# ethz-asl/laser_slam

Hardware: NVIDIA B200
Metric: ICP registrations/s (131072-pt scan vs 524288-pt map, 30 iterations) (higher is better)
Workload: dtype f32

## Files before the change

laser_slam_b200/csrc/ls_api.cu:

```cuda
#include <cstdarg>
#include <cstddef>
#include <cstdio>
#include <cstdlib>
#include <cstring>
#include <string>
#include <utility>
#include <vector>

#include "../../include/ls_b200.h"
#include "ls_kernels.cuh"

using namespace ls;

#define LS_VERSION 100

struct Workspace {
  cudaStream_t stream = nullptr;
  cudaEvent_t ev0 = nullptr, ev1 = nullptr, ev2 = nullptr, ev_launch = nullptr;
  int n_cap = 0, m_cap = 0, cells_cap = 0, tab_cap = 0, hist_cap = 0;
  BuildArrays A{};
  BuildState* bs = nullptr;
  float4 *reading = nullptr, *rd = nullptr;
  float4 *ref_stage = nullptr, *ref_nrm_stage = nullptr;
  float* nrm_raw = nullptr;
// ... 126 lines not shown
    if ((rc = dev_alloc(ctx, &w->ids, (size_t)cap))) return rc;
    if ((rc = dev_alloc(ctx, &w->d2_out, (size_t)cap))) return rc;
    if ((rc = dev_alloc(ctx, &w->A.qkey, (size_t)cap))) return rc;
    if ((rc = dev_alloc(ctx, &w->A.qperm, (size_t)cap))) return rc;
    if ((rc = dev_alloc(ctx, &w->A.rd_s, (size_t)cap))) return rc;
    w->n_cap = cap;
  }
  if (m > w->m_cap) {
    const int cap = m + m / 8 + 1024;
    int rc;
    if ((rc = dev_alloc(ctx, &w->A.sub_pts, (size_t)cap))) return rc;
    if ((rc = dev_alloc(ctx, &w->A.sub_nrm, (size_t)cap))) return rc;
    if ((rc = dev_alloc(ctx, &w->A.srt_pts, (size_t)cap))) return rc;
    if ((rc = dev_alloc(ctx, &w->A.srt_nrm, (size_t)cap))) return rc;
    if ((rc = dev_alloc(ctx, &w->A.pkey, (size_t)cap))) return rc;
    if ((rc = dev_alloc(ctx, &w->ref_stage, (size_t)cap))) return rc;
    if ((rc = dev_alloc(ctx, &w->ref_nrm_stage, (size_t)cap))) return rc;
    int tcap = cap / 17 + 1024;
    const int tmax = (int)((size_t)1536 * 1024 * 1024 / ((size_t)LS_FB3 * 12));
    if (tcap > tmax) tcap = tmax;
    if ((rc = dev_alloc(ctx, &w->A.tab1, (size_t)tcap * LS_FB3))) return rc;
    if ((rc = dev_alloc(ctx, &w->A.cnt1, (size_t)tcap * LS_FB3))) return rc;
    if ((rc = dev_alloc(ctx, &w->A.tab1_cell, (size_t)tcap))) return rc;
    if ((rc = dev_alloc(ctx, &w->A.qtab_local, (size_t)tcap * LS_FB3))) return rc;
    if ((rc = dev_alloc(ctx, &w->A.qtab_total, (size_t)tcap))) return rc;
    CU(cudaMemsetAsync(w->A.cnt1, 0, (size_t)tcap * LS_FB3 * sizeof(uint32_t), w->stream));
    w->stream_dirty = true;
    w->A.tab_cap = tcap;
    w->tab_cap = tcap;
    w->m_cap = cap;
  }
  if (max_cells > w->cells_cap) {
    int rc;
    if ((rc = dev_alloc(ctx, &w->A.top, (size_t)max_cells + 1))) return rc;
    if ((rc = dev_alloc(ctx, &w->A.cnt0, (size_t)max_cells + 1))) return rc;
    if ((rc = dev_alloc(ctx, &w->A.pyr, (size_t)max_cells / 2 + 4096))) return rc;
    if ((rc = dev_alloc(ctx, &w->A.topmask, (size_t)max_cells + 1))) return rc;
    if ((rc = dev_alloc(ctx, &w->A.qtop_start, (size_t)max_cells + 1))) return rc;
    CU(cudaMemsetAsync(w->A.cnt0, 0, ((size_t)max_cells + 1) * sizeof(uint32_t), w->stream));
    w->stream_dirty = true;
    w->cells_cap = max_cells;
  }
  if (max_iter > w->hist_cap) {
    int rc;
    if ((rc = dev_alloc(ctx, &w->T_hist, (size_t)max_iter * 16))) return rc;
    w->hist_cap = max_iter;
  }
  return LS_OK;
}

struct Resolved {
  float cell;
  int split, max_cells;
};

Resolved resolve(const ls_icp_params* p) {
  Resolved r;
  r.cell = p->cell_size > 0.f ? p->cell_size : 1.0f;
  r.split = p->leaf_split > 0 ? (p->leaf_split < 16 ? 16 : p->leaf_split) : 32;
  r.max_cells = p->max_cells > 0 ? p->max_cells : (1 << 22);
  if (r.max_cells > (1 << 22)) r.max_cells = 1 << 22;
  if (r.max_cells < 64) r.max_cells = 64;
  return r;
}

int check_params(ls_ctx* ctx, const ls_icp_params* p) {
  if (!p) return fail(ctx, LS_ERR_ARG, "null params");
  if (p->max_iterations < 1 || p->max_iterations > 100000) return fail(ctx, LS_ERR_ARG, "max_iterations out of range");
  if (!(p->trim_ratio > 0.f) || p->trim_ratio > 1.f) return fail(ctx, LS_ERR_ARG, "trim_ratio must be in (0,1]");
  if (p->use_differential && (p->smooth_length < 1 || p->smooth_length > kMaxSmooth))
    return fail(ctx, LS_ERR_ARG, "smooth_length must be in [1,%d]", kMaxSmooth);
  return LS_OK;
}

void fill_job(Workspace* w, const Parts& parts, const float* T0_host, const float4* reading_dev, int n) {
  BuildJob& J = *w->job_host;
  J.parts = parts;
  J.bs = w->bs;
  J.A = w->A;
  J.m = parts.offset[parts.n_parts];
  J.n = n;
  J.reading = reading_dev;
  J.rd = w->rd;
  std::memcpy(J.T0, T0_host, sizeof(J.T0));
}

int launch_build(ls_ctx* ctx, const BuildJob* jobs_dev, int batch, int m_max, const Resolved& r, cudaStream_t st) {
  const unsigned int B = (unsigned int)batch;
  const int cap = batch > 1 ? ctx->sm_count * 2 : ctx->sm_count * 8;
  const int pb = blocks_for(m_max, 256, cap);
  reset_build_kernel<<<dim3(1, B), 32, 0, st>>>(jobs_dev);
  LAUNCH_CHECK();
  assemble_kernel<<<dim3(pb, B), 256, 0, st>>>(jobs_dev);
  LAUNCH_CHECK();
  setup_kernel<<<dim3(1, B), 32, 0, st>>>(jobs_dev, r.cell, r.max_cells, r.split);
  LAUNCH_CHECK();
  count0_kernel<<<dim3(pb, B), 256, 0, st>>>(jobs_dev);
  LAUNCH_CHECK();
  const int tiles = (r.max_cells + kScanTile - 1) / kScanTile;
  scan_reduce_kernel<<<dim3(tiles, B), kScanThreads, 0, st>>>(jobs_dev);
  LAUNCH_CHECK();
  scan_apply_kernel<<<dim3(tiles, B), kScanThreads, 0, st>>>(jobs_dev);
  LAUNCH_CHECK();
  pyramid1_kernel<<<dim3(blocks_for(r.max_cells / 16 + 1, 256, batch > 1 ? ctx->sm_count : ctx->sm_count * 4), B), 256, 0, st>>>(jobs_dev);
  LAUNCH_CHECK();
  pyramid_up_kernel<<<dim3(1, B), 1024, 0, st>>>(jobs_dev);
  LAUNCH_CHECK();
  count1_kernel<<<dim3(pb, B), 256, 0, st>>>(jobs_dev);
  LAUNCH_CHECK();
  tables_kernel<<<dim3(cap, B), 256, 0, st>>>(jobs_dev);
  LAUNCH_CHECK();
  scatter_kernel<<<dim3(pb, B), 256, 0, st>>>(jobs_dev);
  LAUNCH_CHECK();
  return LS_OK;
}

int launch_reading_sort(ls_ctx* ctx, const BuildJob* jobs_dev, int batch, int n_max, const Resolved& r, cudaStream_t st) {
  const unsigned int B = (unsigned int)batch;
  const int cap = batch > 1 ? ctx->sm_count * 2 : ctx->sm_count * 8;
  const int qb = blocks_for(n_max, 256, cap);
  const int scan_tiles = (r.max_cells + kScanTile - 1) / kScanTile;
  reading_kernel<<<dim3(qb, B), 256, 0, st>>>(jobs_dev);
  LAUNCH_CHECK();
  q_count_kernel<<<dim3(qb, B), 256, 0, st>>>(jobs_dev);
  LAUNCH_CHECK();
  q_tables_kernel<<<dim3(cap, B), 256, 0, st>>>(jobs_dev);
  LAUNCH_CHECK();
  q_scan_reduce_kernel<<<dim3(scan_tiles, B), kScanThreads, 0, st>>>(jobs_dev);
  LAUNCH_CHECK();
  q_scan_apply_kernel<<<dim3(scan_tiles, B), kScanThreads, 0, st>>>(jobs_dev);
  LAUNCH_CHECK();
  q_scatter_kernel<<<dim3(qb, B), 256, 0, st>>>(jobs_dev);
  LAUNCH_CHECK();
  return LS_OK;
}

int enqueue_build(ls_ctx* ctx, Workspace* w, const Parts& parts, const Resolved& r, const float* T0_host) {
  fill_job(w, parts, T0_host, nullptr, 0);
  CU(cudaMemcpyAsync(w->job_dev, w->job_host, sizeof(BuildJob), cudaMemcpyHostToDevice, w->stream));
  return launch_build(ctx, w->job_dev, 1, w->job_host->m, r, w->stream);
}

int upload_normals(ls_ctx* ctx, Workspace* w, const float* normals, int stride, int n, float4* dst) {
  const size_t need = n > 0 ? (stride <= 8 ? (size_t)(n - 1) * (size_t)stride + 3 : (size_t)n * 3) : 0;
  if (need > w->nrm_raw_cap) {
    int rc;
    if ((rc = dev_alloc(ctx, &w->nrm_raw, need + 4096))) return rc;
    w->nrm_raw_cap = need + 4096;
  }
  int dstride = stride;
  if (stride <= 8) {
    CU(cudaMemcpyAsync(w->nrm_raw, normals, need * sizeof(float), cudaMemcpyHostToDevice, w->stream));
  } else {
    CU(cudaMemcpy2DAsync(w->nrm_raw, 3 * sizeof(float), normals, (size_t)stride * sizeof(float), 3 * sizeof(float),
                         (size_t)n, cudaMemcpyHostToDevice, w->stream));
    dstride = 3;
  }
  expand_normals_kernel<<<blocks_for(n, 256, ctx->sm_count * 8), 256, 0, w->stream>>>(w->nrm_raw, dstride, n, dst);
  LAUNCH_CHECK();
  return LS_OK;
}

int fill_problem(ls_ctx* ctx, Workspace* w, const ls_icp_params* prm, int n, const float T0[16], bool want_matches,
                 bool want_hist) {
  IcpProblem& hp = w->hp;
  hp.bs = w->bs;
// ... 929 lines not shown
```

laser_slam_b200/csrc/ls_grid.cuh:

```cuda
#pragma once
#include <cfloat>
#include <climits>
#include <cstring>

#include <vector_types.h>
#include <vector_functions.h>

#include "ls_math.cuh"

#ifndef LS_FB
#define LS_FB 8
#endif
#define LS_FB3 (LS_FB * LS_FB * LS_FB)

namespace ls {

struct Entry {
  uint32_t start;
  int32_t meta;
};

struct Grid {
  float org[3];
  float H0, H1;
// ... 306 lines not shown
    }
  if (b.pos < 0) consider(v.pts, (int)e.start, qx, qy, qz, b);
}

LS_HD Best nn_search(const Grid& g, const GridView& v, float qx, float qy, float qz, int warm_pos, float cap_d2) {
  Best b;
  b.d2 = cap_d2;
  b.idx = INT_MAX;
  b.pos = -1;
  if (g.m <= 0) { b.idx = -1; b.d2 = INFINITY; return b; }
  if (warm_pos >= 0) consider(v.pts, warm_pos, qx, qy, qz, b);
  else seed_query(g, v, qx, qy, qz, b);
  ball_query(g, v, qx, qy, qz, b);
  if (b.pos < 0) { b.idx = -1; b.d2 = INFINITY; }
  return b;
}

#ifndef LS_VK
#define LS_VK 8
#endif
static_assert(LS_VK <= 15, "the list header keeps the candidate count in 4 bits");
#ifndef LS_VL_ABS
#define LS_VL_ABS 0.0f
#endif
#ifndef LS_VL_REL
#define LS_VL_REL 0.5f
#endif
#ifndef LS_VL_SKIN
#define LS_VL_SKIN 4.0f
#endif
#ifndef LS_VL_GATE
#define LS_VL_GATE 1.0f
#endif
struct VLists {
  float4* vq;
  float4* vpts;
  int n;
};

struct Collector {
  float r2;
  int cnt;
  float4* out;
  int stride;
  LS_HD float bound() const { return r2; }
  LS_HD void offer_pt(float d, const float4& c, int p) {
    if (d <= r2) {
      if (cnt < LS_VK) st_state4(out + (size_t)cnt * stride, make_float4(c.x, c.y, c.z, i2f(p)));
      else r2 = -1.0f;
      ++cnt;
    }
  }
};

LS_HD bool vlist_query(const VLists& L, const float4* pts, int i, const float4 v, const float4 c0, float qx, float qy,
                       float qz, float cap_d2, Best& b, float4& cbest) {
  const unsigned int bits = (unsigned int)f2i(v.w);
  if (bits == 0u) return false;
  const int cnt = (int)(bits & 15u);
  const float Rv = i2f((int)(bits & ~15u));
  const float Rc = Rv * 0.999996f - sqrtf(dist2(qx, qy, qz, v.x, v.y, v.z)) * 1.000004f;
  if (!(Rc > 0.0f)) return false;
  b.d2 = cap_d2;
  b.idx = INT_MAX;
  b.pos = -1;
  for (int k = 0; k < cnt; ++k) {
    const float4 c = k == 0 ? c0 : ld_state4(L.vpts + (size_t)k * L.n + i);
    const float d = dist2(qx, qy, qz, c.x, c.y, c.z);
    const int cpos = f2i(c.w);
    if (d < b.d2) {
      b.d2 = d;
      b.pos = cpos;
      cbest = c;
    } else if (d == b.d2) {
      if (b.pos < 0 || f2i(ld_pt(pts + cpos).w) < f2i(ld_pt(pts + b.pos).w)) {
        b.pos = cpos;
        cbest = c;
      }
    }
  }
  return b.d2 * 1.00001f <= Rc * Rc;
}

LS_HD void vlist_build(const Grid& g, const GridView& v, const VLists& L, int i, float qx, float qy, float qz, bool found,
                       float found_d2, float cap_d2, float motion) {
  float Rv;
  if (found) {
    const float want = sqrtf(found_d2);
    const float margin = fmaxf(want * LS_VL_REL, LS_VL_ABS) + 1e-4f;
    if (!(motion * LS_VL_GATE <= margin)) return;
    Rv = want + fminf(margin, fmaxf(0.002f, LS_VL_SKIN * motion));
  } else {
    const float want = sqrtf(cap_d2);
    if (!(motion <= want * 0.125f)) return;
    Rv = want * 1.05f + fminf(want * 0.25f, fmaxf(0.002f, 4.0f * motion));
  }
  if (!(Rv < 3.0e38f)) return;
  Collector c;
  c.r2 = Rv * Rv;
  c.cnt = 0;
  c.out = L.vpts + i;
  c.stride = L.n;
  ball_query(g, v, qx, qy, qz, c);
  float4 head = make_float4(qx, qy, qz, 0.0f);
  if (c.cnt <= LS_VK) head.w = i2f((int)((((unsigned int)f2i(Rv * 0.9999999f)) & ~15u) | (unsigned int)c.cnt));
  st_state4(L.vq + i, head);
}

LS_HDN void knn_search(const Grid& g, const GridView& v, float qx, float qy, float qz, int k, TopK& t) {
  t.reset(k);
  if (g.m <= 0) return;
  const float extent = g.H0 * (float)(g.dim[0] + g.dim[1] + g.dim[2]) + 1.0f;
  float R = g.H1;
  for (int round = 0; round < 64; ++round) {
    t.cap = R * R;
    ball_query(g, v, qx, qy, qz, t);
    if (t.d[k - 1] <= t.cap) break;
    if (R > extent + fabsf(qx - g.org[0]) + fabsf(qy - g.org[1]) + fabsf(qz - g.org[2])) break;
    R = R * 2.0f;
  }
}

LS_HD int top_index(const Grid& g, float x, float y, float z) {
  const int cx = coord_top(x, g.org[0], g.inv0, g.dim[0]);
  const int cy = coord_top(y, g.org[1], g.inv0, g.dim[1]);
  const int cz = coord_top(z, g.org[2], g.inv0, g.dim[2]);
  return (cz * g.dim[1] + cy) * g.dim[0] + cx;
}
LS_HD void top_origin(const Grid& g, int c0, float& lox, float& loy, float& loz) {
  const int cx = c0 % g.dim[0];
  const int cy = (c0 / g.dim[0]) % g.dim[1];
  const int cz = c0 / (g.dim[0] * g.dim[1]);
  lox = cell_lo(g.org[0], cx, g.H0);
  loy = cell_lo(g.org[1], cy, g.H0);
  loz = cell_lo(g.org[2], cz, g.H0);
}
LS_HD int sub_index(float x, float y, float z, float lox, float loy, float loz, float inv) {
  return (coord_sub(z, loz, inv) * LS_FB + coord_sub(y, loy, inv)) * LS_FB + coord_sub(x, lox, inv);
}

LS_HDN void grid_setup(Grid& g, const float* lo, const float* hi, float cell_size, int max_cells, int leaf_split,
                       int m) {
  float H = cell_size > 0.f ? cell_size : 2.0f;
  float ext[3], emax = 0.f, oabs = 0.f;
  for (int a = 0; a < 3; ++a) {
    ext[a] = hi[a] - lo[a];
    if (!(ext[a] >= 0.f)) ext[a] = 0.f;
    emax = fmaxf(emax, ext[a]);
    oabs = fmaxf(oabs, fmaxf(fabsf(lo[a]), fabsf(hi[a])));
  }
  for (int it = 0; it < 40; ++it) {
    double cells = 1.0;
    for (int a = 0; a < 3; ++a) cells *= floor((double)ext[a] / (double)H) + 1.0;
    if (cells <= (double)max_cells) break;
    H = H * 2.0f;
  }
  g.H0 = H;
  g.H1 = H / (float)LS_FB;
  g.inv0 = 1.0f / g.H0;
  g.inv1 = 1.0f / g.H1;
  int n = 1;
  for (int a = 0; a < 3; ++a) {
    g.org[a] = lo[a];
    int d = (int)floorf(ext[a] * g.inv0) + 1;
    if (d < 1) d = 1;
    g.dim[a] = d;
    n *= d;
  }
  g.n_cells0 = n;
  g.margin = (oabs + emax + H) * 1.9073486328125e-06f;
  g.m = m;
  g.leaf_split = leaf_split > 0 ? leaf_split : 32;
  g.n_tab1 = 0;
  g.overflow = 0;
  for (int a = 0; a < 3; ++a) g.pdim[0][a] = g.dim[a];
  g.poff[0] = 0;
  int off = 0, l = 0;
  do {
    ++l;
    for (int a = 0; a < 3; ++a) g.pdim[l][a] = (g.pdim[l - 1][a] + 3) / 4;
    g.poff[l] = off;
    off += g.pdim[l][0] * g.pdim[l][1] * g.pdim[l][2];
  } while ((g.pdim[l][0] > 1 || g.pdim[l][1] > 1 || g.pdim[l][2] > 1) && l < 7);
  g.n_pyr = l;
  g.n_pyr_cells = off;
}

}
```

laser_slam_b200/csrc/ls_kernels.cuh:

```cuda
#pragma once
#include <cuda_runtime.h>
#include <cooperative_groups.h>

#include "ls_grid.cuh"

namespace ls {

constexpr int kMaxParts = 16;
constexpr int kScanTile = 4096;
constexpr int kScanThreads = 512;
#ifndef LS_ICP_THREADS
#define LS_ICP_THREADS 512
#endif
constexpr int kIcpThreads = LS_ICP_THREADS;
constexpr int kIcpCtasPerSm = 1024 / kIcpThreads;
constexpr int kMaxSmooth = 15;
constexpr uint32_t kTag1 = 1u << 31, kKeyMask = (1u << 31) - 1u;

struct Parts {
  int n_parts;
  int offset[kMaxParts + 1];
  const float4* pts[kMaxParts];
  const float4* nrm[kMaxParts];
  float T[kMaxParts][16];
  int identity[kMaxParts];
};

struct BuildState {
  unsigned long long sum[3];
  unsigned int minkey[3], maxkey[3];
  Grid grid;
  float T_pre[16];
  unsigned int tile_sums[1024];
};

struct BuildArrays {
  float4* sub_pts;
  float4* sub_nrm;
  float4* srt_pts;
  float4* srt_nrm;
  uint32_t* pkey;
  Entry* top;
  uint32_t* cnt0;
  Entry* tab1;
  uint32_t* cnt1;
  uint32_t* tab1_cell;
  int tab_cap;
  unsigned long long* pyr;
  unsigned long long* topmask;
  uint32_t* qkey;
  uint32_t* qtop_start;
  uint32_t* qtab_local;
  uint32_t* qtab_total;
  uint32_t* qperm;
  float4* rd_s;
};

struct BuildJob {
  Parts parts;
  BuildState* bs;
  BuildArrays A;
  int m;
  int n;
  const float4* reading;
  float4* rd;
  float T0[16];
};

struct IcpParamsDev {
  int max_iterations;
  float trim_ratio;
  int use_differential;
  float min_diff_rot, min_diff_trans;
  int smooth_length;
};

struct alignas(16) IcpWork {
  unsigned int barrier;
  unsigned int pad0[31];
  unsigned int hist[2][5][2048];
  unsigned long long acc[2][32];
  unsigned int qctr[2];
  float T_out[16];
  int status, iterations, converged, max_iter_reached, last_kept;
  float last_limit;
  int fail_code;
  unsigned int xsignals;
  unsigned int dbg_total, dbg_bin[3], dbg_rem[3];
  double dbg_A[6], dbg_x[6];
};

constexpr int kMaxShards = 8;
struct ShardLink {
  IcpWork* slots;
  IcpWork* peer_slots[kMaxShards];
  unsigned int* flag;
  unsigned int* peer_flag[kMaxShards];
  unsigned int flag_base;
};

struct IcpProblem {
  const BuildState* bs;
  GridView view;
  const float4* nrm;
  const float4* rd;
  int n;
  int* pos;
  float* d2;
  int* ids;
  float* d2_out;
  const uint32_t* qperm;
  VLists lists;
  IcpWork* work;
  int shard_rank, shard_count;
  ShardLink link;
  float* T_hist;
  int want_matches;
  unsigned long long* phase_ns;
  float T0[16];
};

__device__ __forceinline__ unsigned int float_order_key(float f) {
  const unsigned int u = __float_as_uint(f);
  return (u & 0x80000000u) ? ~u : (u | 0x80000000u);
}
__device__ __forceinline__ float float_from_order_key(unsigned int k) {
  const unsigned int u = (k & 0x80000000u) ? (k & 0x7fffffffu) : ~k;
  return __uint_as_float(u);
}

__device__ __forceinline__ long long warp_sum_ll(long long v) {
  unsigned int lo = (unsigned int)(v & 0x1FFFFF);
  unsigned int mid = (unsigned int)((v >> 21) & 0x1FFFFF);
  int hi = (int)(v >> 42);
  lo = __reduce_add_sync(0xffffffffu, lo);
  mid = __reduce_add_sync(0xffffffffu, mid);
  hi = __reduce_add_sync(0xffffffffu, hi);
  return ((long long)hi << 42) + ((long long)mid << 21) + (long long)lo;
}

__global__ void __launch_bounds__(256) assemble_kernel(const BuildJob* __restrict__ jobs) {
  const BuildJob& J = jobs[blockIdx.y];
  const Parts& parts = J.parts;
  float4* __restrict__ sub_pts = J.A.sub_pts;
  float4* __restrict__ sub_nrm = J.A.sub_nrm;
  BuildState* bs = J.bs;
  const int total = parts.offset[parts.n_parts];
  long long s0 = 0, s1 = 0, s2 = 0;
// ... 399 lines not shown
      A.qtab_local[(size_t)t * LS_FB3 + threadIdx.x * per + k] = run;
      run += c[k];
    }
    if (threadIdx.x == 0) A.qtab_total[t] = total;
  }
}

__device__ __forceinline__ unsigned int q_cell_count(const BuildArrays& A, int c) {
  const Entry e = A.top[c];
  return e.meta < 0 ? A.qtab_total[~e.meta] : A.cnt0[c];
}

__global__ void __launch_bounds__(kScanThreads) q_scan_reduce_kernel(const BuildJob* __restrict__ jobs) {
  BuildState* bs = jobs[blockIdx.y].bs;
  const BuildArrays A = jobs[blockIdx.y].A;
  const int n = bs->grid.n_cells0;
  const int base = blockIdx.x * kScanTile;
  if (base >= n) return;
  unsigned int s = 0;
  for (int k = threadIdx.x; k < kScanTile; k += kScanThreads) {
    const int c = base + k;
    if (c < n) s += q_cell_count(A, c);
  }
  s = __reduce_add_sync(0xffffffffu, s);
  __shared__ unsigned int ws[kScanThreads / 32];
  if ((threadIdx.x & 31) == 0) ws[threadIdx.x >> 5] = s;
  __syncthreads();
  if (threadIdx.x == 0) {
    unsigned int t = 0;
    for (int w = 0; w < kScanThreads / 32; ++w) t += ws[w];
    bs->tile_sums[blockIdx.x] = t;
  }
}

__global__ void __launch_bounds__(kScanThreads) q_scan_apply_kernel(const BuildJob* __restrict__ jobs) {
  BuildState* bs = jobs[blockIdx.y].bs;
  const BuildArrays A = jobs[blockIdx.y].A;
  const int n = bs->grid.n_cells0;
  const int base = blockIdx.x * kScanTile;
  if (base >= n) return;
  __shared__ unsigned int ws[kScanThreads / 32];
  __shared__ unsigned int tile_off;
  unsigned int s = 0;
  for (int u = threadIdx.x; u < (int)blockIdx.x; u += kScanThreads) s += bs->tile_sums[u];
  s = __reduce_add_sync(0xffffffffu, s);
  if ((threadIdx.x & 31) == 0) ws[threadIdx.x >> 5] = s;
  __syncthreads();
  if (threadIdx.x == 0) {
    unsigned int t = 0;
    for (int w = 0; w < kScanThreads / 32; ++w) t += ws[w];
    tile_off = t;
  }
  __syncthreads();
  constexpr int per = kScanTile / kScanThreads;
  unsigned int c[per], loc = 0;
  const int first = base + threadIdx.x * per;
#pragma unroll
  for (int k = 0; k < per; ++k) {
    c[k] = (first + k < n) ? q_cell_count(A, first + k) : 0u;
    loc += c[k];
  }
  unsigned int incl = loc;
  const int lane = threadIdx.x & 31, warp = threadIdx.x >> 5;
  for (int o = 1; o < 32; o <<= 1) {
    const unsigned int v = __shfl_up_sync(0xffffffffu, incl, o);
    if (lane >= o) incl += v;
  }
  __syncthreads();
  if (lane == 31) ws[warp] = incl;
  __syncthreads();
  unsigned int woff = 0;
  for (int w = 0; w < warp; ++w) woff += ws[w];
  unsigned int run = tile_off + woff + incl - loc;
#pragma unroll
  for (int k = 0; k < per; ++k) {
    if (first + k < n) A.qtop_start[first + k] = run;
    run += c[k];
  }
}

__global__ void __launch_bounds__(256) q_scatter_kernel(const BuildJob* __restrict__ jobs) {
  const BuildArrays A = jobs[blockIdx.y].A;
  const float4* __restrict__ rd = jobs[blockIdx.y].rd;
  const int n = jobs[blockIdx.y].n;
  for (int i = blockIdx.x * blockDim.x + threadIdx.x; i < n; i += gridDim.x * blockDim.x) {
    const uint32_t k = A.qkey[i];
    uint32_t rank;
    if (k & kTag1) {
      const uint32_t key = k & kKeyMask;
      rank = A.qtop_start[A.tab1_cell[key / (uint32_t)LS_FB3]] + A.qtab_local[key] + atomicSub(&A.cnt1[key], 1u) - 1u;
    } else {
      rank = A.qtop_start[k] + atomicSub(&A.cnt0[k], 1u) - 1u;
    }
    A.rd_s[rank] = __ldg(rd + i);
    A.qperm[rank] = (uint32_t)i;
  }
}

__global__ void shard_slice_kernel(IcpProblem* P, const BuildJob* __restrict__ job, int shard_rank, int shard_count) {
  if (threadIdx.x != 0 || blockIdx.x != 0) return;
  const BuildArrays A = job->A;
  const int n_cells = job->bs->grid.n_cells0, n = job->n;
  auto cut = [&](int s) -> int {
    if (s <= 0) return 0;
    if (s >= shard_count) return n;
    const unsigned int target = (unsigned int)((long long)n * s / shard_count);
    int lo = 0, hi = n_cells;
    while (lo < hi) {
      const int mid = (lo + hi) >> 1;
      if (A.qtop_start[mid] < target) lo = mid + 1;
      else hi = mid;
    }
    return lo < n_cells ? (int)A.qtop_start[lo] : n;
  };
  const int q0 = cut(shard_rank), q1 = cut(shard_rank + 1);
  P->rd += q0;
  P->qperm += q0;
  P->pos += q0;
  P->d2 += q0;
  P->lists.vq += q0;
  P->lists.vpts += q0;
  P->n = q1 - q0;
}

__global__ void __launch_bounds__(256) reading_kernel(const BuildJob* __restrict__ jobs) {
  const BuildState* __restrict__ bs = jobs[blockIdx.y].bs;
  const float4* __restrict__ in = jobs[blockIdx.y].reading;
  float4* __restrict__ out = jobs[blockIdx.y].rd;
  const int n = jobs[blockIdx.y].n;
  __shared__ float T[16];
  if (threadIdx.x < 16) T[threadIdx.x] = bs->T_pre[threadIdx.x];
  __syncthreads();
  for (int i = blockIdx.x * blockDim.x + threadIdx.x; i < n; i += gridDim.x * blockDim.x) {
    const float4 a = __ldg(in + i);
    float4 o;
    xform_point(T, a.x, a.y, a.z, o.x, o.y, o.z);
    o.w = a.w;
    out[i] = o;
  }
}

__global__ void __launch_bounds__(256) transform_kernel(const float* __restrict__ Tg, const float4* __restrict__ in,
                                                        const float4* __restrict__ nin, int n, float4* __restrict__ out,
                                                        float4* __restrict__ nout) {
  __shared__ float T[16];
  if (threadIdx.x < 16) T[threadIdx.x] = Tg[threadIdx.x];
  __syncthreads();
  for (int i = blockIdx.x * blockDim.x + threadIdx.x; i < n; i += gridDim.x * blockDim.x) {
    const float4 a = __ldg(in + i);
    float4 o;
    xform_point(T, a.x, a.y, a.z, o.x, o.y, o.z);
    o.w = a.w;
    out[i] = o;
    if (nin) {
      const float4 b = __ldg(nin + i);
      float4 r;
      rotate_vec(T, b.x, b.y, b.z, r.x, r.y, r.z);
      r.w = 0.f;
      nout[i] = r;
    }
  }
}

__global__ void pack_normals_kernel(const float4* __restrict__ in, int n, float* __restrict__ out3) {
  for (int i = blockIdx.x * blockDim.x + threadIdx.x; i < n; i += gridDim.x * blockDim.x) {
    const float4 a = in[i];
    out3[3 * (size_t)i] = a.x;
    out3[3 * (size_t)i + 1] = a.y;
    out3[3 * (size_t)i + 2] = a.z;
  }
}


__global__ void __launch_bounds__(256) nn_query_kernel(const BuildState* __restrict__ bs, GridView view,
                                                       const float4* __restrict__ rd, int n, int* __restrict__ ids,
                                                       float* __restrict__ d2) {
  __shared__ Grid g;
  if (threadIdx.x == 0) g = bs->grid;
// ... 228 lines not shown
  const float dx = sx - q.x, dy = sy - q.y, dz = sz - q.z;
  e = dx * nn.x;
  float t = dy * nn.y;
  e = e + t;
  t = dz * nn.z;
  e = e + t;
}

constexpr int kPairSlots = 64;
constexpr int kIcpPairBytes = (kIcpThreads / 32) * kPairSlots * 8 * (int)sizeof(float);
__constant__ unsigned char kPairRow[32] = {0, 0, 0, 0, 0, 0, 1, 1, 1, 1, 1, 2, 2, 2, 2, 3, 3, 3, 4, 4, 5, 0, 1, 2, 3, 4, 5, 7, 7, 7, 7, 7};
__constant__ unsigned char kPairCol[32] = {0, 1, 2, 3, 4, 5, 1, 2, 3, 4, 5, 2, 3, 4, 5, 3, 4, 5, 4, 5, 5, 6, 6, 6, 6, 6, 6, 7, 7, 7, 7, 7};

struct PairQueue {
  float* recs;
  int head, cnt;
  long long acc;
};

__device__ __noinline__ long long consume_pairs(const float* recs, int head, int count, long long acc) {
  const int lane = threadIdx.x & 31;
  const int ro = kPairRow[lane], co = kPairCol[lane];
  const float scale = lane < 27 ? 4194304.0f : 1.0f;
#pragma unroll 4
  for (int j = 0; j < count; ++j) {
    const float* r = recs + ((head + j) & (kPairSlots - 1)) * 8;
    const float a = r[ro], b = r[co], sg = r[7];
    long long v = __float2ll_rn((a * b) * scale);
    if (sg < 0.f) v = -v;
    acc += v;
  }
  return acc;
}

template <int site>
__device__ __forceinline__ void push_pairs(const IcpProblem& P, PairQueue& Q, int sign, float sx, float sy, float sz,
                                           const float4 q, int pos) {
  const unsigned int m = __ballot_sync(0xffffffffu, sign != 0);
  if (m == 0u) return;
#ifdef LS_DEBUG_PAIRS
  if (sign && (pos < 0 || pos >= P.bs->grid.m)) {
    printf("[ls] push_pairs: sign %d pos %d site %d block %d thread %d q.w %d\n", sign, pos, site, (int)blockIdx.x, (int)threadIdx.x, __float_as_int(q.w));
    sign = 0;
  }
#endif
  if (sign) {
    float f[6], e;
    residual_terms(sx, sy, sz, q, __ldg(P.nrm + pos), f, e);
    const int slot = (Q.head + Q.cnt + __popc(m & ((1u << (threadIdx.x & 31)) - 1u))) & (kPairSlots - 1);
    float4* r = reinterpret_cast<float4*>(Q.recs + slot * 8);
    r[0] = make_float4(f[0], f[1], f[2], f[3]);
    r[1] = make_float4(f[4], f[5], e, (float)sign);
  }
  Q.cnt += __popc(m);
  __syncwarp();
  if (Q.cnt >= 32) {
    Q.acc = consume_pairs(Q.recs, Q.head, 32, Q.acc);
    Q.head = (Q.head + 32) & (kPairSlots - 1);
    Q.cnt -= 32;
    __syncwarp();
  }
}

__device__ __forceinline__ void drain_pairs(PairQueue& Q, unsigned long long* slab) {
  if (Q.cnt > 0) {
    Q.acc = consume_pairs(Q.recs, Q.head, Q.cnt, Q.acc);
    Q.head = (Q.head + Q.cnt) & (kPairSlots - 1);
    Q.cnt = 0;
  }
  const int lane = threadIdx.x & 31;
  if (lane < 28) slab[lane] = (unsigned long long)Q.acc;
  Q.acc = 0ll;
  __syncwarp();
}

__device__ __noinline__ void phase_a_search(const Grid* gp, const IcpProblem* Pp, const float* T_iter, const float* T_prev,
                                            int i, float cap, SelHists* H, unsigned int pred_bin1, unsigned int pred_pref12) {
  if (i < 0) return;
  const Grid& g = *gp;
  const IcpProblem& P = *Pp;
  const float4 r = __ldg(P.rd + i);
  float sx, sy, sz;
  xform_point(T_iter, r.x, r.y, r.z, sx, sy, sz);
  const int warm = __ldcg(P.pos + i);
  const Best b = nn_search(g, P.view, sx, sy, sz, warm, cap);
  phase_a_record(P, i, b, H, pred_bin1, pred_pref12);
  if (T_prev) {
    float px, py, pz;
    xform_point(T_prev, r.x, r.y, r.z, px, py, pz);
    vlist_build(g, P.view, P.lists, i, sx, sy, sz, b.pos >= 0, b.d2, cap, sqrtf(dist2(sx, sy, sz, px, py, pz)));
  }
}

template <int site>
__device__ __forceinline__ void push_searched(const IcpProblem& P, PairQueue& Q, const float* T_iter, int j, float acc_limit) {
  if (!(acc_limit >= 0.0f)) return;
  float d = INFINITY;
  if (j >= 0) d = __ldcg(P.d2 + j);
  const bool keep = d <= acc_limit;
  if (__ballot_sync(0xffffffffu, keep) == 0u) return;
  float4 q = make_float4(0.f, 0.f, 0.f, 0.f);
  float sx = 0.f, sy = 0.f, sz = 0.f;
  int pos = -1;
  if (keep) {
    pos = __ldcg(P.pos + j);
    const float4 r = __ldg(P.rd + j);
    xform_point(T_iter, r.x, r.y, r.z, sx, sy, sz);
    q = __ldg(P.view.pts + pos);
  }
  push_pairs<site>(P, Q, keep ? 1 : 0, sx, sy, sz, q, pos);
}

__device__ __noinline__ void final_match(const Grid* gp, const IcpProblem* Pp, const float* T, int i) {
  if (i < 0) return;
  const IcpProblem& P = *Pp;
  const float4 r = __ldg(P.rd + i);
  float sx, sy, sz;
  xform_point(T, r.x, r.y, r.z, sx, sy, sz);
  const Best b = nn_search(*gp, P.view, sx, sy, sz, __ldcg(P.pos + i), INFINITY);
  const uint32_t orig = __ldg(P.qperm + i);
  P.d2_out[orig] = b.d2;
  P.ids[orig] = b.idx;
}

__device__ __forceinline__ void flush_slabs(unsigned long long (*acc_w)[28], unsigned long long* gacc) {
  __syncthreads();
  if (threadIdx.x < 28) {
    unsigned long long t = 0ull;
#pragma unroll
    for (int w = 0; w < kIcpThreads / 32; ++w) t += acc_w[w][threadIdx.x];
    if (t != 0ull) atomicAdd(&gacc[threadIdx.x], t);
  }
  __syncthreads();
}

__device__ __forceinline__ void flush_hist(const unsigned int* hs, int nbins, unsigned int* gh) {
  for (int k = threadIdx.x; k < nbins; k += kIcpThreads) {
    const unsigned int v = hs[k];
    if (v) atomicAdd(&gh[k], v);
  }
}

__global__ void __launch_bounds__(kIcpThreads, kIcpCtasPerSm)
icp_kernel(const IcpProblem* __restrict__ probs, int ctas_per_problem, IcpParamsDev prm, int dynamic) {
  const int pi = blockIdx.x / ctas_per_problem;
  const int cta = blockIdx.x - pi * ctas_per_problem;
  const IcpProblem& P = probs[pi];
  IcpWork* W = P.work;
  const bool xg = P.shard_count > 1;
  IcpWork* X = xg ? P.link.slots + P.shard_rank : W;
  const IcpWork* S0 = xg ? P.link.slots : W;
  const int n_slots = xg ? P.shard_count : 1;
  const unsigned int G = (unsigned int)ctas_per_problem;
  unsigned int xepoch = 0;
  const int tid = threadIdx.x, lane = tid & 31;

  __shared__ Grid g;
  __shared__ float T_iter[16], T_last[16];
  __shared__ SelHists hs;
  __shared__ unsigned long long acc_w[kIcpThreads / 32][28];
  __shared__ SelectOut sel;
  __shared__ unsigned int ws[kIcpThreads / 32];
  __shared__ double qh[kMaxSmooth + 2][4];
  __shared__ double th[kMaxSmooth + 2][3];
  __shared__ int flag_stop, flag_status;
  __shared__ int miss_buf[kIcpThreads / 32][64];
  extern __shared__ __align__(16) float pair_buf[];

  if (tid == 0) {
    g = P.bs->grid;
    for (int i = 0; i < 16; ++i) T_iter[i] = (i % 5 == 0) ? 1.f : 0.f;
    quat_from_T(T_iter, qh[0]);
    th[0][0] = th[0][1] = th[0][2] = 0.0;
    flag_stop = 0;
    flag_status = 0;
  }
  __syncthreads();
  PairQueue Q;
  Q.recs = pair_buf + (tid >> 5) * (kPairSlots * 8);
  Q.head = 0;
  Q.cnt = 0;
  Q.acc = 0ll;

  const int n = P.n;
  int chunk = (n + (int)G - 1) / (int)G;
  chunk = (chunk + 31) & ~31;
  const int q_begin = min(n, cta * chunk), q_end = min(n, q_begin + chunk);

  for (int i = q_begin + tid; i < q_end; i += kIcpThreads) {
    __stcg(P.pos + i, -1);
    __stcg(P.lists.vq + i, make_float4(0.f, 0.f, 0.f, 0.f));
  }

  float cap = 0.04f;
  int redo = 0;
  unsigned int epoch = 0;
  constexpr int kHistOff = (int)(offsetof(IcpWork, hist) / 4), kAccOff = (int)(offsetof(IcpWork, acc) / 4);
  auto meet = [&](int off0, int n0, int off1, int n1, int off2, int n2) {
    if (xg) shard_exchange(P, X, cta, G, epoch, xepoch, off0, n0, off1, n1, off2, n2);
    else problem_barrier(&X->barrier, G, epoch);
  };
  problem_barrier(&X->barrier, G, epoch);
  int hist_count = 1;
  int iter = 0, converged = 0, max_reached = 0, last_kept = 0;
  float last_limit = 0.f;
  unsigned int pred_bin1 = kNoPrediction, pred_pref12 = kNoPrediction;
  float acc_limit = -1.0f;

  for (;;) {
    const int par = iter & 1;
    LS_STAMP(0);
    for (int k = tid; k < (int)(sizeof(SelHists) / 4); k += kIcpThreads) reinterpret_cast<unsigned int*>(&hs)[k] = 0u;
    __syncthreads();
    {
      const float* T_prev = iter >= 1 ? T_last : nullptr;
      int* mq = miss_buf[tid >> 5];
      int n_miss = 0;
      int next = q_begin + (tid & ~31);
      for (;;) {
        int base;
        if (dynamic) {
          unsigned int bb = 0;
          if (lane == 0) bb = atomicAdd(&W->qctr[par], 32u);
          bb = __shfl_sync(0xffffffffu, bb, 0);
          if (bb >= (unsigned int)n) break;
          base = (int)bb;
        } else {
          if (next >= q_end) break;
          base = next;
          next += kIcpThreads;
        }
        const int i = base + lane;
        bool valid = i < (dynamic ? n : q_end);
        if (redo && valid) valid = !(__ldcg(P.d2 + i) < INFINITY);
        bool hit = false;
        Best b;
        b.d2 = INFINITY; b.idx = INT_MAX; b.pos = -1;
        float4 c = make_float4(0.f, 0.f, 0.f, 0.f);
        float sx = 0.f, sy = 0.f, sz = 0.f;
        if (valid) {
          const float4 r = __ldg(P.rd + i);
          const float4 v = __ldcg(P.lists.vq + i);
          const float4 c0 = __ldcg(P.lists.vpts + i);
          xform_point(T_iter, r.x, r.y, r.z, sx, sy, sz);
          hit = vlist_query(P.lists, P.view.pts, i, v, c0, sx, sy, sz, cap, b, c);
          if (hit) phase_a_record(P, i, b, &hs, pred_bin1, pred_pref12);
        }
        push_pairs<0>(P, Q, (hit && b.pos >= 0 && b.d2 <= acc_limit) ? 1 : 0, sx, sy, sz, c, b.pos);
        const unsigned int mm = __ballot_sync(0xffffffffu, valid && !hit);
        if (mm) {
          if (valid && !hit) mq[n_miss + __popc(mm & ((1u << lane) - 1u))] = i;
          n_miss += __popc(mm);
          __syncwarp();
          if (n_miss >= 32) {
            n_miss -= 32;
            const int j = mq[n_miss + lane];
            __syncwarp();
            phase_a_search(&g, &P, T_iter, T_prev, j, cap, &hs, pred_bin1, pred_pref12);
            push_searched<1>(P, Q, T_iter, j, acc_limit);
          }
        }
      }
      if (n_miss > 0) {
        __syncwarp();
        const int j = lane < n_miss ? mq[lane] : -1;
        phase_a_search(&g, &P, T_iter, T_prev, j, cap, &hs, pred_bin1, pred_pref12);
        __syncwarp();
        push_searched<2>(P, Q, T_iter, j, acc_limit);
      }
    }
    drain_pairs(Q, acc_w[tid >> 5]);
    flush_slabs(acc_w, X->acc[par]);
    flush_hist(hs.h1, 1024, X->hist[par][0]);
    if (pred_bin1 != kNoPrediction) {
      flush_hist(hs.h2, 2048, X->hist[par][3]);
// ... 196 lines not shown
```

Before: 1229.

## Fuse NN search with verlet-list build and seed warm positions from grid cells

Replaces the separate nearest-neighbour search followed by a second ball query for the verlet list with one ball query. That query tracks the best match and collects list candidates at the same time, with the list radius shrinking as the best distance improves, then compacts any entries outside the final radius. The query scatter kernel now writes an initial warm-start map position from each query's grid cell instead of -1, which gives the first search a nearby seed. Costs: the collector uses more registers, the ball query runs when motion is infinite, and list entries can overflow and be trimmed.

```diff
diff --git a/laser_slam_b200/csrc/ls_api.cu b/laser_slam_b200/csrc/ls_api.cu
--- a/laser_slam_b200/csrc/ls_api.cu
+++ b/laser_slam_b200/csrc/ls_api.cu
@@ -232,6 +232,7 @@
   J.n = n;
   J.reading = reading_dev;
   J.rd = w->rd;
+  J.pos = w->pos;
   std::memcpy(J.T0, T0_host, sizeof(J.T0));
 }
 
diff --git a/laser_slam_b200/csrc/ls_grid.cuh b/laser_slam_b200/csrc/ls_grid.cuh
--- a/laser_slam_b200/csrc/ls_grid.cuh
+++ b/laser_slam_b200/csrc/ls_grid.cuh
@@ -412,20 +412,29 @@
   return b.d2 * 1.00001f <= Rc * Rc;
 }
 
-LS_HD void vlist_build(const Grid& g, const GridView& v, const VLists& L, int i, float qx, float qy, float qz, bool found,
-                       float found_d2, float cap_d2, float motion) {
+LS_HD float vlist_radius(bool found, float d2, float cap_d2, float motion) {
   float Rv;
   if (found) {
-    const float want = sqrtf(found_d2);
+    const float want = sqrtf(d2);
     const float margin = fmaxf(want * LS_VL_REL, LS_VL_ABS) + 1e-4f;
-    if (!(motion * LS_VL_GATE <= margin)) return;
+    if (!(motion * LS_VL_GATE <= margin)) return -1.0f;
     Rv = want + fminf(margin, fmaxf(0.002f, LS_VL_SKIN * motion));
   } else {
     const float want = sqrtf(cap_d2);
-    if (!(motion <= want * 0.125f)) return;
+    if (!(motion <= want * 0.125f)) return -1.0f;
     Rv = want * 1.05f + fminf(want * 0.25f, fmaxf(0.002f, 4.0f * motion));
   }
-  if (!(Rv < 3.0e38f)) return;
+  return Rv < 3.0e38f ? Rv : -1.0f;
+}
+
+LS_HD float vlist_header(float Rv, int cnt) {
+  return i2f((int)((((unsigned int)f2i(Rv * 0.9999999f)) & ~15u) | (unsigned int)cnt));
+}
+
+LS_HD void vlist_build(const Grid& g, const GridView& v, const VLists& L, int i, float qx, float qy, float qz, bool found,
+                       float found_d2, float cap_d2, float motion) {
+  const float Rv = vlist_radius(found, found_d2, cap_d2, motion);
+  if (!(Rv > 0.0f)) return;
   Collector c;
   c.r2 = Rv * Rv;
   c.cnt = 0;
@@ -433,8 +442,90 @@
   c.stride = L.n;
   ball_query(g, v, qx, qy, qz, c);
   float4 head = make_float4(qx, qy, qz, 0.0f);
-  if (c.cnt <= LS_VK) head.w = i2f((int)((((unsigned int)f2i(Rv * 0.9999999f)) & ~15u) | (unsigned int)c.cnt));
+  if (c.cnt <= LS_VK) head.w = vlist_header(Rv, c.cnt);
   st_state4(L.vq + i, head);
+}
+
+struct BestList {
+  float d2;
+  int idx;
+  int pos;
+  float r2;
+  float dmax;
+  float ddrop;
+  int cnt;
+  float motion;
+  float4* out;
+  int stride;
+  LS_HD float bound() const { return fmaxf(d2, r2); }
+  LS_HD void offer_pt(float d, const float4& c, int p) {
+    const int i = f2i(c.w);
+    if (d < d2 || (d == d2 && i < idx)) {
+      d2 = d;
+      idx = i;
+      pos = p;
+      if (r2 >= 0.0f) {
+        const float r = vlist_radius(true, d, 0.0f, motion);
+        r2 = r > 0.0f ? r * r : -1.0f;
+      }
+    }
+    if (d <= r2) {
+      if (cnt < LS_VK) {
+        st_state4(out + (size_t)cnt * stride, make_float4(c.x, c.y, c.z, i2f(p)));
+        ++cnt;
+        dmax = fmaxf(dmax, d);
+      } else {
+        ddrop = fminf(ddrop, d);
+      }
+    }
+  }
+};
+
+LS_HD Best nn_search_list(const Grid& g, const GridView& v, const VLists& L, int i, float qx, float qy, float qz,
+                          int warm_pos, float cap_d2, float motion) {
+  Best s;
+  s.d2 = cap_d2;
+  s.idx = INT_MAX;
+  s.pos = -1;
+  if (g.m <= 0) { s.idx = -1; s.d2 = INFINITY; return s; }
+  if (warm_pos >= 0) consider(v.pts, warm_pos, qx, qy, qz, s);
+  else seed_query(g, v, qx, qy, qz, s);
+  BestList b;
+  b.d2 = s.d2;
+  b.idx = s.idx;
+  b.pos = s.pos;
+  float r = vlist_radius(true, s.d2, cap_d2, motion);
+  if (s.pos < 0) r = fmaxf(r, vlist_radius(false, 0.0f, cap_d2, motion));
+  b.r2 = r > 0.0f ? r * r : -1.0f;
+  b.dmax = 0.0f;
+  b.ddrop = INFINITY;
+  b.cnt = 0;
+  b.motion = motion;
+  b.out = L.vpts + i;
+  b.stride = L.n;
+  ball_query(g, v, qx, qy, qz, b);
+  s.d2 = b.d2;
+  s.idx = b.idx;
+  s.pos = b.pos;
+  if (s.pos < 0) { s.idx = -1; s.d2 = INFINITY; }
+  float Rv = vlist_radius(b.pos >= 0, b.d2, cap_d2, motion);
+  if (!(Rv > 0.0f)) return s;
+  if (b.ddrop < INFINITY) Rv = fminf(Rv, sqrtf(b.ddrop) * 0.999999f);
+  const float r2 = Rv * Rv;
+  int cnt = b.cnt;
+  if (b.dmax > r2) {
+    int w = 0;
+    for (int k = 0; k < b.cnt; ++k) {
+      const float4 c = ld_state4(L.vpts + (size_t)k * L.n + i);
+      if (dist2(qx, qy, qz, c.x, c.y, c.z) <= r2) {
+        if (w != k) st_state4(L.vpts + (size_t)w * L.n + i, c);
+        ++w;
+      }
+    }
+    cnt = w;
+  }
+  st_state4(L.vq + i, make_float4(qx, qy, qz, vlist_header(Rv, cnt)));
+  return s;
 }
 
 LS_HDN void knn_search(const Grid& g, const GridView& v, float qx, float qy, float qz, int k, TopK& t) {
diff --git a/laser_slam_b200/csrc/ls_kernels.cuh b/laser_slam_b200/csrc/ls_kernels.cuh
--- a/laser_slam_b200/csrc/ls_kernels.cuh
+++ b/laser_slam_b200/csrc/ls_kernels.cuh
@@ -64,6 +64,7 @@
   int n;
   const float4* reading;
   float4* rd;
+  int* pos;
   float T0[16];
 };
 
@@ -629,6 +630,7 @@
 __global__ void __launch_bounds__(256) q_scatter_kernel(const BuildJob* __restrict__ jobs) {
   const BuildArrays A = jobs[blockIdx.y].A;
   const float4* __restrict__ rd = jobs[blockIdx.y].rd;
+  int* __restrict__ pos = jobs[blockIdx.y].pos;
   const int n = jobs[blockIdx.y].n;
   for (int i = blockIdx.x * blockDim.x + threadIdx.x; i < n; i += gridDim.x * blockDim.x) {
     const uint32_t k = A.qkey[i];
@@ -641,6 +643,15 @@
     }
     A.rd_s[rank] = __ldg(rd + i);
     A.qperm[rank] = (uint32_t)i;
+    int warm = -1;
+    if (k & kTag1) {
+      const Entry e1 = A.tab1[k & kKeyMask];
+      warm = (int)(e1.meta != 0 ? e1.start : A.top[A.tab1_cell[(k & kKeyMask) / (uint32_t)LS_FB3]].start);
+    } else {
+      const Entry e0 = A.top[k];
+      if (e0.meta > 0) warm = (int)e0.start;
+    }
+    pos[rank] = warm;
   }
 }
 
@@ -1035,14 +1046,15 @@
   const float4 r = __ldg(P.rd + i);
   float sx, sy, sz;
   xform_point(T_iter, r.x, r.y, r.z, sx, sy, sz);
-  const int warm = __ldcg(P.pos + i);
-  const Best b = nn_search(g, P.view, sx, sy, sz, warm, cap);
-  phase_a_record(P, i, b, H, pred_bin1, pred_pref12);
+  float motion = INFINITY;
   if (T_prev) {
     float px, py, pz;
     xform_point(T_prev, r.x, r.y, r.z, px, py, pz);
-    vlist_build(g, P.view, P.lists, i, sx, sy, sz, b.pos >= 0, b.d2, cap, sqrtf(dist2(sx, sy, sz, px, py, pz)));
-  }
+    motion = sqrtf(dist2(sx, sy, sz, px, py, pz));
+  }
+  const int warm = __ldcg(P.pos + i);
+  const Best b = nn_search_list(g, P.view, P.lists, i, sx, sy, sz, warm, cap, motion);
+  phase_a_record(P, i, b, H, pred_bin1, pred_pref12);
 }
 
 template <int site>
@@ -1140,10 +1152,8 @@
   chunk = (chunk + 31) & ~31;
   const int q_begin = min(n, cta * chunk), q_end = min(n, q_begin + chunk);
 
-  for (int i = q_begin + tid; i < q_end; i += kIcpThreads) {
-    __stcg(P.pos + i, -1);
+  for (int i = q_begin + tid; i < q_end; i += kIcpThreads)
     __stcg(P.lists.vq + i, make_float4(0.f, 0.f, 0.f, 0.f));
-  }
 
   float cap = 0.04f;
   int redo = 0;
```

Result: slower. 1137 (median of 6 runs) (-7.5%).
